# hkchengrex/Cutie

Hardware: AMD Instinct MI355X
Metric: frames/sec (480p, 3 objects) (higher is better)
Workload: dtype bf16

## Files before the change

### cutie_amd/csrc/conv_pc.hip

```cpp
#include "conv_common.h"

typedef __amdgpu_buffer_rsrc_t rsrc_t;
#define PC_WORD3 0x00020000
#define PC_RECORDS 0x7fffffff
#define PC_OOB 0x80000000u
#define LDS_PTR(p) ((__attribute__((address_space(3))) void*)(p))
#define PC_WAIT_VM(N) __builtin_amdgcn_s_waitcnt(((N) & 15) | (((N) >> 4) << 14) | (7 << 4) | (15 << 8))
#define PC_WAIT_LGKM0() __builtin_amdgcn_s_waitcnt(15 | (3 << 14) | (7 << 4) | (0 << 8))
#define PC_BARRIER() { asm volatile("" ::: "memory"); __builtin_amdgcn_s_barrier(); asm volatile("" ::: "memory"); }
#ifdef PC_ABL_NO_LOOPBAR
#define PC_LOOP_BARRIER() { asm volatile("" ::: "memory"); }
#else
#define PC_LOOP_BARRIER() PC_BARRIER()
#endif
#ifdef PC_ABL_NO_WAIT
#define PC_LOOP_WAIT_VM(N) ((void)0)
#else
#define PC_LOOP_WAIT_VM(N) PC_WAIT_VM(N)
#endif
#ifdef PC_ABL_SAME_TILE
#define PC_SAME_TILE_GUARD(...)
#else
#define PC_SAME_TILE_GUARD(...) __VA_ARGS__
#endif
#ifdef PC_ABL_NO_DMA
#define PC_DMA(...) ((void)0)
#else
#define PC_DMA(...) __builtin_amdgcn_raw_ptr_buffer_load_lds(__VA_ARGS__)
#endif

__device__ __forceinline__ rsrc_t pc_rsrc(const void* base) {
    return __builtin_amdgcn_make_buffer_rsrc(const_cast<void*>(base), 0, PC_RECORDS, PC_WORD3);
}

typedef short pc_s16x2 __attribute__((ext_vector_type(2)));
__device__ __forceinline__ unsigned pc_relu2(unsigned w) {
    return __builtin_bit_cast(unsigned, __builtin_elementwise_max(__builtin_bit_cast(pc_s16x2, w), (pc_s16x2){0, 0}));
}

__device__ __forceinline__ int pc_wrow(int R, bool pair) {
    if (!pair) return R;
    const int ii = R & 15, alo = (R >> 4) & 1;
    return (R & ~31) | ((ii >> 2) << 3) | (alo << 2) | (ii & 3);
}

#define PC_HT(TH, TW) ((TH) * 256 + (TW))
template <int BM, int BN, int NS, int HT>
constexpr int pc_lds_bytes(int NPW) {
    if (HT == 0) return NS * (BM + BN) * 128;
    const int TH = HT >> 8, TW = HT & 255, npiece = ((TH + 2) * (TW + 2) + 7) / 8, nxp = (npiece + NPW - 1) / NPW;
    return 2 * nxp * NPW * 1024 + NS * BN * 128;
}

template <int NCH>
__device__ __forceinline__ void pc_finish(const ConvParams& p, float (&v)[NCH], int m, int ch0, bool vec_ok, bool have_res,
                                          const unsigned (&rpre)[NCH / 2], float (&stored)[NCH]) {
#ifdef PC_ABL_FIXED_EPI
    {
#pragma unroll
        for (int r = 0; r < NCH; ++r) v[r] = fmaxf(v[r], 0.f);
        bf16_t* yp = reinterpret_cast<bf16_t*>(p.y) + (long)m * p.ldy + ch0;
        unsigned o[NCH / 2];
#pragma unroll
        for (int r = 0; r < NCH / 2; ++r) o[r] = pack_bf2(v[2 * r], v[2 * r + 1]);
        if constexpr (NCH == 8) *reinterpret_cast<uint4*>(yp) = make_uint4(o[0], o[1], o[NCH / 2 - 2], o[NCH / 2 - 1]);
        else *reinterpret_cast<uint2*>(yp) = make_uint2(o[0], o[1]);
        return;
    }
#endif
    const int act = (p.flags >> CUTIE_ACT_SHIFT) & 7;
    const bool out_f32 = p.flags & CUTIE_F_OUT_F32;
    const bool full = ch0 + NCH <= p.Cout;
    if (p.res) {
        if (have_res) {
#pragma unroll
            for (int r = 0; r < NCH / 2; ++r) { v[2 * r] += __uint_as_float(rpre[r] << 16); v[2 * r + 1] += __uint_as_float(rpre[r] & 0xffff0000u); }
        } else {
            const int mres = conv_res_row(p, m);
            const bf16_t* rp = p.res + (long)mres * p.ldr + ch0;
            if (full && vec_ok) {
                unsigned rr[NCH / 2];
                if constexpr (NCH == 8) { const uint4 t = *reinterpret_cast<const uint4*>(rp); rr[0] = t.x; rr[1] = t.y; rr[NCH / 2 - 2] = t.z; rr[NCH / 2 - 1] = t.w; }
                else { const uint2 t = *reinterpret_cast<const uint2*>(rp); rr[0] = t.x; rr[1] = t.y; }
#pragma unroll
// ... 148 lines not shown
                    }
                }
            }
        }
        if (GAPJ) {
            int c; bool writer;
            const long long tot = pc_colsum16<NCH>(gs, l15, c, writer);
            if (writer) pc_gap_add(p, gap_obj, chbase + a * (PAIR ? 32 : 16) + c, tot);
        }
    }
}

template <int BM, int BN, int WM, int WN, int NPW, int NS, int HT, bool TAPS, bool RELU, bool TWO, int KP = 1>
__global__ __launch_bounds__((WM * WN + NPW) * 64) void conv_pc_kernel(ConvParams p) {
#if __HIP_DEVICE_COMPILE__
    if (p.flags & CUTIE_F_PRIO) __builtin_amdgcn_s_setprio(1);
    constexpr bool HALO = HT > 0;
    constexpr int TH = HALO ? (HT >> 8) : 1, TW = HALO ? (HT & 255) : 1;
    constexpr int NC = WM * WN, NTC = NC * 64;
    constexpr int TM = BM / WM / 16, TN = BN / WN / 16;
    constexpr bool PAIR = (TN % 2) == 0;
    constexpr int NCH = PAIR ? 8 : 4, TNP = PAIR ? TN / 2 : TN;
    constexpr int NXI = HALO ? 1 : BM / 8 / NPW;
    constexpr int NWI = BN / 8 / NPW;
    constexpr int LPT = HALO ? NWI : NXI + NWI;
    constexpr int PH = TH + 2, PW = TW + 2;
    constexpr int NPIECE = (PH * PW + 7) / 8, NXP = (NPIECE + NPW - 1) / NPW, XBUF = NXP * NPW * 1024;
    constexpr int WSTAGE = BN * 128, STAGE = HALO ? WSTAGE : (BM + BN) * 128;
    constexpr int WBASE = HALO ? 2 * XBUF : 0;
    constexpr bool PRE_RES = TM * TNP <= 4;
    static_assert(TM >= 1 && TN >= 1 && BM % (WM * 16) == 0 && BN % (WN * 16) == 0 && NWI >= 1 && NWI * 8 * NPW == BN && NS >= 2 && NS <= 8, "bad tile");
    static_assert(HALO || (NXI >= 1 && NXI * 8 * NPW == BM), "bad stream tile");
    static_assert(!HALO || (TH * TW <= BM && TH * TW > BM - 16 * WM && (NS == 3 || NS == 4) && NXP <= 11 - NS && NXP <= 8), "bad halo tile");
    static_assert(KP == 1 || (KP == 2 && (NS == 4 || NS == 6)), "pair steps: a ring of 2 or 3 pairs");
    constexpr int NP = NS / 2;
    extern __shared__ __attribute__((aligned(16))) u32x4 pc_smem[];
    char* const lds = reinterpret_cast<char*>(pc_smem);
    const int tid = threadIdx.x, lane = tid & 63, l15 = lane & 15, l4 = lane >> 4;
    const int wave = __builtin_amdgcn_readfirstlane(tid >> 6);
    TL_DECL(lds + pc_lds_bytes<BM, BN, NS, HT>(NPW))
    TL(0)
    conv_preload_args(p);
    TL(10)
    const int nb = gridDim.x * gridDim.y;
    int logical;
    {
        const int id = blockIdx.y * gridDim.x + blockIdx.x;
        const int xcd = id & 7, kq = id >> 3, q = nb >> 3, r = nb & 7;
        logical = (xcd < r ? xcd * (q + 1) : r * (q + 1) + (xcd - r) * q) + kq;
    }
    const int mt = logical / (int)gridDim.y;
    const int n0 = (logical - mt * (int)gridDim.y) * BN;
    int m0 = 0, bimg = 0, ty0 = 0, tx0 = 0;
    if (HALO) {
        const int tiles_x = (p.W + TW - 1) / TW, tiles_y = (p.H + TH - 1) / TH, per = tiles_x * tiles_y;
        bimg = mt / per;
        const int r = mt - bimg * per, ty = r / tiles_x;
        ty0 = ty * TH;
        tx0 = (r - ty * tiles_x) * TW;
    } else {
        m0 = mt * BM;
    }
    if (p.zero) {
        const int nthr = (NC + NPW) * 64;
        for (int z = (blockIdx.y * gridDim.x + blockIdx.x) * nthr + tid; z < p.nzero; z += gridDim.x * gridDim.y * nthr) p.zero[z] = 0ull;
    }
    const int nslice = p.Cin / 64;
#ifdef PC_ABL_NO_LOOP
    const int nk = 0;
#else
    const int nk = HALO ? nslice * 9 : p.KH * p.KW * nslice;
#endif

// ... 140 lines not shown
#undef PCS_WPIECE
#undef PCS_XPIECE
        } else {
            unsigned xo1[NXP], xo2[NXP];
#pragma unroll
            for (int i = 0; i < NXP; ++i) {
                const int pp = (pw + NPW * i) * 8 + lr;
                const int py = pp / PW, px = pp - py * PW;
                const int gy = ty0 - 1 + py, gx = tx0 - 1 + px;
                const bool ok = pp < PH * PW && (unsigned)gy < (unsigned)p.H && (unsigned)gx < (unsigned)p.W;
                const unsigned pix = (unsigned)((bimg * p.H + gy) * p.W + gx);
                const unsigned kc = (unsigned)(((lane & 7) ^ (pp & 7)) * 16);
                xo1[i] = ok ? pix * (unsigned)(p.ldx1 * 2) + kc : PC_OOB;
                xo2[i] = TWO ? (ok ? pix * (unsigned)(p.ldx2 * 2) + kc : PC_OOB) : 0u;
            }
            const rsrc_t rx1 = pc_rsrc(p.x1), rx2 = TWO ? pc_rsrc(p.x2) : rx1;
            const int cin2 = p.Cin * 2;
#define PCH_XPIECE(I, SL)                                                                                      \
    {                                                                                                          \
        const bool f_ = !TWO || (SL) * 64 < p.C1;                                                              \
        const int so_ = (f_ ? (SL) * 64 : (SL) * 64 - p.C1) * 2;                                               \
        PC_DMA(f_ ? rx1 : rx2, LDS_PTR(lds + ((SL) & 1) * XBUF + (pw + NPW * (I)) * 1024), 16, f_ ? xo1[I] : xo2[I], so_, 0, 0); \
    }
            int wsl = 0, wtap = 0, wld = 0;
            unsigned wso = 0;
#define PCH_WTILE()                                                                                            \
    {                                                                                                          \
        _Pragma("unroll") for (int i = 0; i < NWI; ++i) PC_DMA(rw, LDS_PTR(lds + wld + wdst + i * 1024), 16, woff[i], wso, 0, 0); \
        wld = wld == (NS - 1) * WSTAGE ? 0 : wld + WSTAGE;                                                     \
        ++wtap; PC_SAME_TILE_GUARD(wso += (unsigned)cin2;)                                                     \
        if (wtap == 9) { wtap = 0; ++wsl; PC_SAME_TILE_GUARD(wso = (unsigned)(wsl * 128);) }                                       \
    }
            TL(1)
#pragma unroll
            for (int s = 0; s < NS - 1; ++s)
                if (s < nk) PCH_WTILE()
#pragma unroll
            for (int i = 0; i < NXP; ++i) PCH_XPIECE(i, 0)
            PC_WAIT_VM(0);
            TL(2)
            PC_BARRIER()
            if constexpr (KP == 1) {
            int sl = 0, tap = 0;
            int xprev = 0;
            int kt = 0;
            for (; kt < nk - (NS - 1); ++kt) {
                TL(3)
                const int xp = (sl + 1 < nslice && tap < NXP) ? 1 : 0;
                if (xp) {
                    switch (tap) {
                        case 0: if constexpr (NXP > 0) PCH_XPIECE(0, sl + 1) break;
                        case 1: if constexpr (NXP > 1) PCH_XPIECE(NXP > 1 ? 1 : 0, sl + 1) break;
                        case 2: if constexpr (NXP > 2) PCH_XPIECE(NXP > 2 ? 2 : 0, sl + 1) break;
                        case 3: if constexpr (NXP > 3) PCH_XPIECE(NXP > 3 ? 3 : 0, sl + 1) break;
                        case 4: if constexpr (NXP > 4) PCH_XPIECE(NXP > 4 ? 4 : 0, sl + 1) break;
                        case 5: if constexpr (NXP > 5) PCH_XPIECE(NXP > 5 ? 5 : 0, sl + 1) break;
                        case 6: if constexpr (NXP > 6) PCH_XPIECE(NXP > 6 ? 6 : 0, sl + 1) break;
                        default: if constexpr (NXP > 7) PCH_XPIECE(NXP > 7 ? 7 : 0, sl + 1) break;
                    }
                }
                PCH_WTILE()
                TL(4)
                const int xin = NS == 3 ? xp : xp + xprev;
                if (xin == 0) { PC_LOOP_WAIT_VM((NS - 2) * NWI); } else if (xin == 1) { PC_LOOP_WAIT_VM((NS - 2) * NWI + 1); } else { PC_LOOP_WAIT_VM((NS - 2) * NWI + 2); }
                TL(5)
                PC_LOOP_BARRIER()
                xprev = xp;
                ++tap;
                if (tap == 9) { tap = 0; ++sl; }
            }
            for (; kt < nk; ++kt) {
                PC_WAIT_VM(0);
                PC_LOOP_BARRIER()
            }
            } else {
// ... 96 lines not shown
            for (int a = 0; a < TNP; ++a) {
                const int ch0 = n0 + cn0 + a * (PAIR ? 32 : 16) + l4 * NCH;
#pragma unroll
                for (int r = 0; r < NCH / 2; ++r) rpre[b][a][r] = 0u;
                if (have_res && mval[b] && ch0 + NCH <= p.Cout) {
                    const int mres = pc_res_row(p, mrow[b]);
                    const bf16_t* rp = p.res + (long)mres * p.ldr + ch0;
                    if constexpr (NCH == 8) { const uint4 t = *reinterpret_cast<const uint4*>(rp); rpre[b][a][0] = t.x; rpre[b][a][1] = t.y; rpre[b][a][NCH / 2 - 2] = t.z; rpre[b][a][NCH / 2 - 1] = t.w; }
                    else { const uint2 t = *reinterpret_cast<const uint2*>(rp); rpre[b][a][0] = t.x; rpre[b][a][1] = t.y; }
                }
            }
    }
    TL(12)
    const int c0 = l4 << 4, c1 = (4 + l4) << 4;
    const int swl = (l15 & 7) << 4;
    int rdw0, rdx0 = 0;
    rdw0 = (HALO ? 0 : BM * 128) + (cn0 + l15) * 128;
    if (!HALO) rdx0 = (pm0 + l15) * 128;
    f32x4 acc[TN][TM];
#pragma unroll
    for (int a = 0; a < TN; ++a)
#pragma unroll
        for (int b = 0; b < TM; ++b) acc[a][b] = (f32x4){0.f, 0.f, 0.f, 0.f};

#ifdef PC_ABL_NO_MFMA
#define PC_MFMA(AF, BF, ACC) ACC[0] += __uint_as_float(__builtin_bit_cast(u32x4, AF).x ^ __builtin_bit_cast(u32x4, BF).y)
#else
#define PC_MFMA(AF, BF, ACC) ACC = __builtin_amdgcn_mfma_f32_16x16x32_bf16(AF, BF, ACC, 0, 0, 0)
#endif
#define PC_RELU4(V) { V.x = pc_relu2(V.x); V.y = pc_relu2(V.y); V.z = pc_relu2(V.z); V.w = pc_relu2(V.w); }
    int rd = 0;
    int sl = 0, tap = 0, toff = 0;
    TL(1)
    PC_BARRIER()
    TL(2)
    for (int kt = 0; kt < nk; ++kt) {
        TL(3)
        u32x4 x0[TM], x1[TM];
        bf16x8 w0[TN], w1[TN];
#ifdef PC_ABL_NO_READ
#pragma unroll
        for (int a = 0; a < TN; ++a) { u32x4 v = {(unsigned)rd + a, (unsigned)lane, 5u, 1u}; w0[a] = __builtin_bit_cast(bf16x8, v); v.w = 2u; w1[a] = __builtin_bit_cast(bf16x8, v); }
#pragma unroll
        for (int b = 0; b < TM; ++b) { x0[b] = (u32x4){(unsigned)rd + b, (unsigned)lane, 3u, 1u}; x1[b] = (u32x4){(unsigned)rd + b, (unsigned)lane, 3u, 2u}; }
#else
        const char* const wst = lds + WBASE + rd + rdw0;
#pragma unroll
        for (int a = 0; a < TN; ++a) {
            w0[a] = __builtin_bit_cast(bf16x8, *reinterpret_cast<const u32x4*>(wst + a * 2048 + (c0 ^ swl)));
            w1[a] = __builtin_bit_cast(bf16x8, *reinterpret_cast<const u32x4*>(wst + a * 2048 + (c1 ^ swl)));
        }
        if (HALO) {
            const char* const xs = lds + (sl & 1) * XBUF;
#pragma unroll
            for (int b = 0; b < TM; ++b) {
                const int pp = xbase[b] + toff;
                const int sw = (pp & 7) << 4;
                x0[b] = *reinterpret_cast<const u32x4*>(xs + pp * 128 + (c0 ^ sw));
                x1[b] = *reinterpret_cast<const u32x4*>(xs + pp * 128 + (c1 ^ sw));
            }
        } else {
            const char* const xs = lds + rd + rdx0;
#pragma unroll
            for (int b = 0; b < TM; ++b) {
                x0[b] = *reinterpret_cast<const u32x4*>(xs + b * 2048 + (c0 ^ swl));
                x1[b] = *reinterpret_cast<const u32x4*>(xs + b * 2048 + (c1 ^ swl));
            }
        }
#endif
        if (RELU) {
#pragma unroll
            for (int b = 0; b < TM; ++b) { PC_RELU4(x0[b]) PC_RELU4(x1[b]) }
        }
#pragma unroll
        for (int a = 0; a < TN; ++a)
#pragma unroll
            for (int b = 0; b < TM; ++b) PC_MFMA(w0[a], __builtin_bit_cast(bf16x8, x0[b]), acc[a][b]);
#pragma unroll
        for (int a = 0; a < TN; ++a)
#pragma unroll
            for (int b = 0; b < TM; ++b) PC_MFMA(w1[a], __builtin_bit_cast(bf16x8, x1[b]), acc[a][b]);
        TL(4)
        if (KP == 1 || (kt & 1) || kt == nk - 1) {
            PC_WAIT_LGKM0();
            PC_LOOP_BARRIER()
        }
        rd = rd == (NS - 1) * STAGE ? 0 : rd + STAGE;
        if (HALO) {
            ++tap;
            toff += (tap == 3 || tap == 6) ? PW - 2 : 1;
            if (tap == 9) { tap = 0; toff = 0; ++sl; }
        }
    }
    TLE(5)
#ifdef PC_ABL_NO_EPILOGUE
    if (acc[0][0][0] != 12345.678f) { TL_DUMP(logical, nb, NC + NPW) return; }
#endif
    int gap_obj = bimg;
    bool gap_one = true;
    if (p.gap && !HALO) {
        const int mf = m0 + pm0, ml = min(mf + BM / WM - 1, p.M - 1);
        const float rd = __builtin_amdgcn_rcpf((float)p.OHW);
        gap_obj = pc_div(min(mf, p.M - 1), p.OHW, rd);
        gap_one = pc_div(ml, p.OHW, rd) == gap_obj;
    }
#ifndef PC_ABL_GENERIC_EPI
    {
        const int act_ = (p.flags >> CUTIE_ACT_SHIFT) & 7;
        const bool gapfast = p.gap && gap_one && !act_ && !p.res && !out_f32;
        if (vec_ok && n0 + BN <= p.Cout && (!p.gap || gapfast) && act_ <= CUTIE_ACT_RELU && !(out_f32 && (act_ || p.res))) {
            const int chbase = n0 + cn0 + l4 * NCH;
#define PC_FAST(RL, F, RS) pc_epilogue_fast<NCH, TM, TNP, PAIR, RL, F, RS, PRE_RES>(p, acc, bias, mrow, mval, chbase, rpre)
            if (gapfast) pc_epilogue_fast<NCH, TM, TNP, PAIR, false, false, false, PRE_RES, true>(p, acc, bias, mrow, mval, chbase, rpre, gap_obj, l15);
            else if (out_f32) PC_FAST(false, true, false);
            else if (p.res) { if (act_) PC_FAST(true, false, true); else PC_FAST(false, false, true); }
            else { if (act_) PC_FAST(true, false, false); else PC_FAST(false, false, false); }
#undef PC_FAST
            TLE(6)
            TL_DUMP(logical, nb, NC + NPW)
            return;
        }
    }
#endif
#pragma unroll
    for (int a = 0; a < TNP; ++a) {
// ... 36 lines not shown
                            for (int pass = 0; pass < 2; ++pass) {
                                const int oo = pass ? o2 : o1;
                                if (pass && !rest) break;
                                long long part[NCH];
#pragma unroll
                                for (int r = 0; r < NCH; ++r) part[r] = (live && ob == oo) ? pc_gapfx(st[r]) : 0;
                                int c; bool writer;
                                const long long tot = pc_colsum16<NCH>(part, l15, c, writer);
                                if (writer) pc_gap_add(p, oo, ch0 + c, tot);
                            }
                        }
                    }
                }
            }
#endif
        }
#ifndef PC_ABL_FIXED_EPI
        if (p.gap && gap_one) {
            int c; bool writer;
            const long long tot = pc_colsum16<NCH>(gsum, l15, c, writer);
            if (writer) pc_gap_add(p, gap_obj, n0 + cn0 + a * (PAIR ? 32 : 16) + l4 * NCH + c, tot);
        }
#endif
    }
    TLE(6)
    TL_DUMP(logical, nb, NC + NPW)
#undef PC_RELU4
#undef PC_MFMA
#endif
}

template <int BM, int BN, int WM, int WN, int NPW, int NS, int HT, bool TAPS, bool RELU, bool TWO, int KP>
static int launch_pc3(const ConvParams& p, hipStream_t s) {
    constexpr int lds = pc_lds_bytes<BM, BN, NS, HT>(NPW) + TL_BYTES;
    static_assert(lds <= 160 * 1024, "LDS");
    static bool attr_set = false;
    if (!attr_set) {
        if (lds > 65536 && hipFuncSetAttribute(reinterpret_cast<const void*>(conv_pc_kernel<BM, BN, WM, WN, NPW, NS, HT, TAPS, RELU, TWO, KP>),
                                               hipFuncAttributeMaxDynamicSharedMemorySize, lds) != hipSuccess) {
            cutie_set_error("conv pc tile: cannot raise the dynamic LDS limit to %d bytes", lds);
            return -2;
        }
        attr_set = true;
    }
    unsigned gx;
    if (HT > 0) {
        constexpr int TH = HT > 0 ? (HT >> 8) : 1, TW = HT > 0 ? (HT & 255) : 1;
        gx = (unsigned)(p.B * ((p.H + TH - 1) / TH) * ((p.W + TW - 1) / TW));
    } else {
        gx = (unsigned)((p.M + BM - 1) / BM);
    }
    hipLaunchKernelGGL((conv_pc_kernel<BM, BN, WM, WN, NPW, NS, HT, TAPS, RELU, TWO, KP>), dim3(gx, (unsigned)((p.Cout + BN - 1) / BN)),
                       dim3((WM * WN + NPW) * 64), lds, s, p);
    return (int)hipGetLastError();
}

template <int BM, int BN, int WM, int WN, int NPW, int NS, int HT, int KP = 1>
static int launch_pc(ConvParams p, hipStream_t s) {
    const long x1_bytes = (long)p.B * p.H * p.W * p.ldx1 * 2, x2_bytes = p.C2 ? (long)p.B * p.H * p.W * p.ldx2 * 2 : 0;
    const long gy = (p.Cout + BN - 1) / BN, w_bytes = gy * BN * (long)p.Kpad * 2;
    if (p.Cin % 64 || (p.C2 && p.C1 % 64) || p.KH > 5 || p.KW > 5 || p.splitk != 1 || p.Kpad < p.KH * p.KW * p.Cin ||
        x1_bytes >= PC_RECORDS - 8192 || x2_bytes >= PC_RECORDS - 8192 || w_bytes >= PC_RECORDS - 8192) {
        cutie_set_error("conv pc tile: needs Cin %% 64 == 0 (C1 too for two sources), KH, KW <= 5, no split-K, operands < 2 GiB "
                        "(Cin=%d C1=%d Kpad=%d k=%dx%d splitk=%d)", p.Cin, p.C1, p.Kpad, p.KH, p.KW, p.splitk);
        return -2;
    }
    if (HT > 0 && (p.KH != 3 || p.KW != 3 || p.stride != 1 || p.pad != 1 || p.OH != p.H || p.OW != p.W)) {
        cutie_set_error("conv pc halo tile: needs 3x3 / stride 1 / pad 1 (k=%dx%d stride=%d pad=%d)", p.KH, p.KW, p.stride, p.pad);
        return -2;
    }
    p.Kslice = p.KH * p.KW * p.Cin;
    const bool relu = p.flags & CUTIE_F_RELU_IN, two = p.C2 != 0, taps = p.pad > 0 || p.KH * p.KW > 1;
#define PC_GO(T_, R_, W_) return launch_pc3<BM, BN, WM, WN, NPW, NS, HT, T_, R_, W_, KP>(p, s)
    if constexpr (HT > 0) {
        if (relu) { if (two) PC_GO(true, true, true); PC_GO(true, true, false); }
        if (two) PC_GO(true, false, true);
        PC_GO(true, false, false);
    } else {
        if (taps) {
            if (relu) { if (two) PC_GO(true, true, true); PC_GO(true, true, false); }
            if (two) PC_GO(true, false, true);
            PC_GO(true, false, false);
        }
        if (relu) { if (two) PC_GO(false, true, true); PC_GO(false, true, false); }
        if (two) PC_GO(false, false, true);
        PC_GO(false, false, false);
    }
#undef PC_GO
}

int launch_conv_pc(const ConvParams& p, int tile, hipStream_t s) {
    switch (tile) {
        case 100: return launch_pc<64, 64, 2, 2, 4, 3, 0>(p, s);
#ifndef PC_QUICK
        case 101: return launch_pc<64, 64, 2, 2, 4, 4, 0>(p, s);
        case 102: return launch_pc<32, 64, 2, 2, 4, 4, 0>(p, s);
        case 103: return launch_pc<128, 64, 2, 2, 4, 3, 0>(p, s);
        case 104: return launch_pc<64, 128, 2, 2, 4, 3, 0>(p, s);
        case 105: return launch_pc<128, 128, 2, 2, 4, 3, 0>(p, s);
        case 106: return launch_pc<128, 128, 2, 2, 8, 3, 0>(p, s);
        case 107: return launch_pc<64, 64, 2, 2, 8, 3, 0>(p, s);
        case 108: return launch_pc<128, 128, 2, 4, 8, 3, 0>(p, s);
        case 109: return launch_pc<32, 64, 2, 2, 4, 6, 0>(p, s);
        case 110: return launch_pc<96, 64, 2, 2, 4, 3, 0>(p, s);
        case 111: return launch_pc<96, 128, 2, 2, 4, 3, 0>(p, s);
#endif
        case 120: return launch_pc<64, 64, 2, 2, 4, 3, PC_HT(8, 8)>(p, s);
#ifndef PC_QUICK
        case 121: return launch_pc<64, 64, 2, 2, 4, 3, PC_HT(4, 16)>(p, s);
        case 122: return launch_pc<128, 64, 2, 2, 4, 3, PC_HT(8, 16)>(p, s);
        case 123: return launch_pc<128, 128, 2, 2, 4, 3, PC_HT(8, 16)>(p, s);
        case 124: return launch_pc<64, 128, 2, 2, 4, 3, PC_HT(8, 8)>(p, s);
        case 125: return launch_pc<32, 64, 2, 2, 4, 3, PC_HT(4, 8)>(p, s);
        case 126: return launch_pc<128, 128, 2, 4, 8, 3, PC_HT(8, 16)>(p, s);
        case 127: return launch_pc<64, 128, 2, 2, 4, 3, PC_HT(4, 16)>(p, s);
        case 129: return launch_pc<96, 64, 2, 2, 4, 3, PC_HT(10, 9)>(p, s);
        case 130: return launch_pc<32, 64, 2, 2, 4, 3, PC_HT(5, 6)>(p, s);
        case 131: return launch_pc<64, 128, 2, 2, 4, 3, PC_HT(6, 9)>(p, s);
        case 132: return launch_pc<64, 64, 2, 2, 4, 3, PC_HT(6, 9)>(p, s);
        case 133: return launch_pc<96, 128, 2, 2, 4, 3, PC_HT(10, 9)>(p, s);
        case 134: return launch_pc<320, 64, 4, 2, 8, 3, PC_HT(20, 16)>(p, s);
        case 140: return launch_pc<64, 64, 2, 2, 4, 4, 0, 2>(p, s);
        case 141: return launch_pc<96, 64, 2, 2, 4, 4, 0, 2>(p, s);
        case 142: return launch_pc<96, 64, 2, 2, 4, 6, 0, 2>(p, s);
        case 143: return launch_pc<32, 64, 2, 2, 4, 4, 0, 2>(p, s);
        case 144: return launch_pc<128, 64, 2, 2, 4, 4, 0, 2>(p, s);
        case 145: return launch_pc<96, 64, 2, 2, 4, 4, PC_HT(10, 9), 2>(p, s);
        case 146: return launch_pc<128, 64, 2, 2, 4, 4, PC_HT(8, 16), 2>(p, s);
        case 147: return launch_pc<32, 64, 2, 2, 4, 4, PC_HT(5, 6), 2>(p, s);
#endif
        default: cutie_set_error("conv: bad pc tile id %d", tile); return -2;
    }
}
```

### cutie_amd/model/plans.py

```python
import math
import os

import numpy as np
import torch

from .. import _lib
from .. import ops as O
from ..ops import Dyn
from .param_spec import resnet_layers

BF16, F32 = torch.bfloat16, torch.float32


class Act:
    __slots__ = ('t', 'B', 'H', 'W', 'C', 'ld')

    def __init__(self, t, B, H, W, C, ld=None):
        self.t, self.B, self.H, self.W, self.C, self.ld = t, B, H, W, C, (C if ld is None else ld)


def positional_encoding(h, w, dim_total, scale, temperature):
    dim = int(math.ceil(dim_total / 4) * 2)
    inv_freq = 1.0 / (temperature ** (torch.arange(0, dim, 2).float() / dim))
    py = torch.arange(h, dtype=torch.float32)
# ... 281 lines not shown
            fl = int(arr['flags'][n])
            key = O.conv_tile_key(M, cout, cin, int(i[11]), int(i[13]), fl & O.F_RELU_IN, fl & O.F_OUT_F32, int(i[1]), int(i[2]))
            best = cache.get(key)
            twin = self.korder_ref and int(i[0]) % self.korder_ref == 0
            kref = self.kref.get(n)
            twin = twin or kref is not None
            if twin:
                M1 = M // self.korder_ref if kref is None else M * kref // int(i[0])
                key1 = (M1,) + key[1:]
                ref = cache.get(key1) or (O.static_tile(M1, cout, cin, int(i[11]), int(i[4]), cout1=int(i[17]) == O.COUT1_TILE), 1)
                want = O.korder_class(*ref)
                if isinstance(want, str) and cache.get(key + (want,)) is not None:
                    best = cache[key + (want,)]
                if best is None or O.korder_class(*best) != want:
                    best = (int(i[17]), 1) if O.korder_class(int(i[17]), int(i[19])) == want else tuple(ref)
                assert O.korder_class(*best) == want, (key, best, ref)
            if best is None and not getattr(self.eng, 'autotune', AUTOTUNE):
                continue
            if best is None:
                one = arr[n:n + 1].copy()
                best, best_t = (int(i[17]), 1), None
                cands = O.tile_candidates(M, cout, cin, int(i[16]),
                                          geom=dict(kh=int(i[11]), stride=int(i[13]), pad=int(i[14]), W=int(i[2]), c2=int(i[4])))
                if int(i[4]) or arr['p'][n, 4]:
                    cands = [t for t in cands if t != O.COUT1_TILE]
                for t in cands:
                    for sk in O.splitk_candidates(M, cout, int(i[16]), t):
                        one['i'][0, 17], one['i'][0, 19] = t, sk
                        ms = min(ex.time_ops(one, TUNE_ITERS) for _ in range(TUNE_REPS))
                        if best_t is None or ms < best_t:
                            best, best_t = (t, sk), ms
                cache[key] = best
                tuned_any = True
            apply = True
            if (best[0] in O.DMA_TILES or best[0] in O.PC_TILES) and not O.dma_tiles_enabled():
                apply = False
            if (arr['p'][n, 7] or arr['p'][n, 8]) and best[0] not in O.DMA_TILES and best[0] not in O.PC_TILES:
                apply = False
            if apply:
                arr['i'][n, 17], arr['i'][n, 19] = best
            if twin:
                assert O.korder_class(int(arr['i'][n, 17]), int(arr['i'][n, 19])) == want, (key, int(arr['i'][n, 17]), int(arr['i'][n, 19]), want)
        ol.wire_next_weights()
        self.tuned = True
        if tuned_any:
            save_tile_cache(cache)

    def conv(self, wname, x, *, name=None, out=None, stride=1, pad=None, x2=None, res=None, res_bcast=False,
             relu_in=False, act=O.ACT_NONE, out_f32=False, ldy=None, gap_acc=None, zero=None, persistent=False, res_group=None):
        w = self.eng.w[wname]
        if pad is None:
            pad = (w.kh - 1) // 2
        OH = (x.H + 2 * pad - w.kh) // stride + 1
        OW = (x.W + 2 * pad - w.kw) // stride + 1
        if out is None:
            t = self.buf(name or wname, (x.B, OH, OW, w.cout), F32 if out_f32 else BF16, persistent=persistent)
            out = Act(t, x.B, OH, OW, w.cout, w.cout if ldy is None else ldy)
        else:
            assert out.B == x.B and out.H == OH and out.W == OW and out.C == w.cout, (wname, out.B, out.H, out.W, out.C, OH, OW, w.cout)
        if res is not None:
            assert res.C == w.cout and res.H == OH and res.W == OW

        def emit(s0, s1, zero):
            whole = s0 == 0 and s1 == x.B
            cut = (lambda a, elem: a.t) if whole else (lambda a, elem: _objects_from(a, s0, elem))
            return self.ol.conv(cut(x, 2), w, cut(out, 4 if out_f32 else 2), B=s1 - s0, H=x.H, W=x.W, C1=x.C, ldx1=x.ld, OH=OH, OW=OW, ldy=out.ld, stride=stride,
# ... 456 lines not shown
```

### cutie_amd/model/weights.py

```python
import torch

BN_EPS = 1e-5


class PackedConv:
    __slots__ = ('weight', 'bias', 'cout', 'cin_padded', 'kh', 'kw', 'kpad', 'cin_real')

    def __init__(self, weight, bias, cout, cin_padded, kh, kw, kpad, cin_real=None):
        self.weight, self.bias, self.cout, self.cin_padded = weight, bias, cout, cin_padded
        self.kh, self.kw, self.kpad = kh, kw, kpad
        self.cin_real = cin_padded if cin_real is None else cin_real


class PackedLinear:
    __slots__ = ('weight', 'bias', 'n', 'kd')

    def __init__(self, weight, bias, n, kd):
        self.weight, self.bias, self.n, self.kd = weight, bias, n, kd


def fold_bn(w, sd, bn):
    g, b = sd[bn + '.weight'].float(), sd[bn + '.bias'].float()
    m, v = sd[bn + '.running_mean'].float(), sd[bn + '.running_var'].float()
    s = g / torch.sqrt(v + BN_EPS)
    return w * s.view(-1, 1, 1, 1), b - m * s


def pack_conv(w, bias, device, segs=None):
    w = w.float()
    cout, cin, kh, kw = w.shape
    if segs is None:
        segs = [(cin, -(-cin // 8) * 8)]
    assert sum(r for r, _ in segs) == cin
    parts, c0 = [], 0
    for real, padded in segs:
        assert padded % 8 == 0 and padded >= real
        part = w[:, c0:c0 + real]
        if padded > real:
            part = torch.cat([part, torch.zeros(cout, padded - real, kh, kw)], 1)
        parts.append(part)
        c0 += real
    w = torch.cat(parts, 1)
    cin_p = w.shape[1]
    k = kh * kw * cin_p
    kpad = -(-k // 128) * 128
    coutpad = -(-cout // 128) * 128
    flat = w.permute(0, 2, 3, 1).reshape(cout, k)
    packed = torch.zeros(coutpad, kpad)
    packed[:cout, :k] = flat
    return PackedConv(packed.to(torch.bfloat16).to(device).contiguous(),
                      None if bias is None else bias.float().to(device).contiguous(), cout, cin_p, kh, kw, kpad, cin_real=cin)


def pack_linear(w, bias, device):
    w = w.float()
    n, kd = w.shape
    assert kd % 8 == 0
    return PackedLinear(w.to(torch.bfloat16).to(device).contiguous(),
                        None if bias is None else bias.float().to(device).contiguous(), n, kd)


def linear_as_conv(w, bias, device):
    return pack_conv(w.float().view(w.shape[0], w.shape[1], 1, 1), bias, device)


def out_proj_blob(w):
    assert w.cout == 256 and w.kh == 1 and w.kw == 1 and w.cin_padded == 256 and w.bias is not None
    return torch.cat([w.weight[:256, :256].contiguous().view(torch.uint8).reshape(-1), w.bias.contiguous().view(torch.uint8).reshape(-1)]).contiguous()
```

### cutie_amd/ops.py

```python
import os

import numpy as np
import torch

from . import _lib

NI, NF, NP = 24, 6, 16
OP_DTYPE = np.dtype([('kind', '<i4'), ('flags', '<i4'), ('i', '<i4', (NI,)), ('f', '<f4', (NF,)), ('p', '<u8', (NP,))])
assert OP_DTYPE.itemsize == _lib.OP_STRUCT_SIZE

(CONV, MAXPOOL, IMG_PREP, UPSAMPLE2X_ADD, AREA_DOWN, MASK_DOWN, GAP, ECA_APPLY, GRU, SEG_AGG, UP4_SOFTMAX,
 MASK_MERGE, AGG_SOFTMAX, LINEAR, LAYERNORM, QUERY_INIT, AUX_MASK, ATTN_Q2P, ATTN_SELF, ATTN_P2Q, SUMMARIZE,
 ADD_PE, KEY_PREP, AFF_SCORE, AFF_SELECT, AFF_READOUT, MEMSET32, COPY2D, AXPY, USAGE_TICK, RANK_SELECT,
 GATHER_ROWS, CONSOL_AFF, CONSOL_READ, CAST, PROB_TO_ID, RESIZE, FLIP_W, AREA_DOWN3, QFFN, STEM, BANK_WRITE) = range(1, 43)

KIND_NAMES = {}
for _n in ('CONV MAXPOOL IMG_PREP UPSAMPLE2X_ADD AREA_DOWN MASK_DOWN GAP ECA_APPLY GRU SEG_AGG UP4_SOFTMAX MASK_MERGE '
           'AGG_SOFTMAX LINEAR LAYERNORM QUERY_INIT AUX_MASK ATTN_Q2P ATTN_SELF ATTN_P2Q SUMMARIZE ADD_PE KEY_PREP '
           'AFF_SCORE AFF_SELECT AFF_READOUT MEMSET32 COPY2D AXPY USAGE_TICK RANK_SELECT GATHER_ROWS CONSOL_AFF '
           'CONSOL_READ CAST PROB_TO_ID RESIZE FLIP_W AREA_DOWN3 QFFN STEM').split():
    KIND_NAMES[globals()[_n]] = _n

F_RELU_IN, F_OUT_F32, F_RES_BCAST = 1, 2, 4
F_PRIO, F_AFF_PRIO = 256, 64
F_TILE_OFF = 128 if os.environ.get('CUTIE_AMD_COUT1_TILE', '1') in ('', '0') else 0
ACT_NONE, ACT_RELU, ACT_SIGMOID, ACT_SQ1 = 0, 1, 2, 3
ACT_SHIFT = 4
AREA_RT = 8 if os.environ.get('CUTIE_AMD_AREA_R', '1') in ('', '0') else 0
GRU_SCALAR = 1 if os.environ.get('CUTIE_AMD_GRU4', '1') in ('', '0') else 0
KEYPREP_LOOP = 2 if os.environ.get('CUTIE_AMD_KEYPREP_LOOP', '0') not in ('', '0') else 0
UP4_LANES = 16 if os.environ.get('CUTIE_AMD_UP4_SHARED', '1') in ('', '0') else 0
SELECT_COARSE = 2 if os.environ.get('CUTIE_AMD_SELECT_FINE', '1') in ('', '0') else 0
UP4_RTK = 8 if os.environ.get('CUTIE_AMD_UP4_KC', '1') in ('', '0') else 0

TILES = {0: (128, 128, 32), 1: (128, 64, 32), 2: (64, 64, 32), 3: (256, 16, 32), 4: (64, 128, 32),
         5: (64, 64, 64), 6: (64, 128, 64), 7: (128, 128, 64), 8: (64, 64, 128), 9: (32, 64, 64),
         10: (128, 64, 64), 11: (32, 64, 128), 12: (32, 128, 64),
         13: (64, 64, 64), 14: (128, 64, 64), 15: (64, 128, 64), 16: (128, 128, 64), 17: (64, 64, 128), 18: (128, 128, 32),
         20: (64, 64, 64), 21: (64, 64, 128), 22: (32, 64, 128), 23: (128, 64, 64), 24: (64, 128, 64), 25: (128, 128, 64),
         26: (32, 64, 64), 27: (64, 64, 64), 28: (32, 64, 64), 29: (64, 128, 32), 30: (64, 64, 32)}
TILE_WK = {20: 2, 21: 2, 22: 2, 23: 2, 24: 2, 25: 2, 26: 2, 27: 4, 28: 4, 29: 2, 30: 2}

DMA_TILES = {60: (128, 128, 64), 61: (128, 128, 64), 62: (128, 128, 64), 63: (128, 64, 64), 64: (64, 128, 64), 65: (64, 64, 64),
             66: (64, 64, 64), 67: (32, 64, 64), 68: (256, 128, 64), 69: (32, 128, 64), 70: (128, 128, 64), 71: (128, 64, 64),
             72: (64, 64, 64), 73: (64, 64, 64), 74: (64, 64, 64), 75: (32, 64, 64), 76: (128, 64, 64), 77: (64, 128, 64), 78: (32, 128, 64),
             80: (64, 64, 128), 81: (64, 64, 128), 82: (32, 64, 128), 83: (32, 64, 128), 84: (64, 128, 128), 85: (128, 64, 128),
             86: (96, 64, 64), 87: (96, 64, 64), 88: (64, 64, 64), 89: (64, 64, 64)}


PC_TILES = {100: (64, 64, 64), 101: (64, 64, 64), 102: (32, 64, 64), 103: (128, 64, 64), 104: (64, 128, 64), 105: (128, 128, 64),
            106: (128, 128, 64), 107: (64, 64, 64), 108: (128, 128, 64), 109: (32, 64, 64), 110: (96, 64, 64), 111: (96, 128, 64),
            120: (64, 64, 64), 121: (64, 64, 64), 122: (128, 64, 64), 123: (128, 128, 64), 124: (64, 128, 64), 125: (32, 64, 64),
            126: (128, 128, 64), 127: (64, 128, 64), 129: (96, 64, 64), 130: (32, 64, 64), 131: (64, 128, 64),
            132: (64, 64, 64), 133: (96, 128, 64), 134: (320, 64, 64),
            140: (64, 64, 64), 141: (96, 64, 64), 142: (96, 64, 64), 143: (32, 64, 64), 144: (128, 64, 64),
            145: (96, 64, 64), 146: (128, 64, 64), 147: (32, 64, 64)}
PC_HALO = {120: (8, 8), 121: (4, 16), 122: (8, 16), 123: (8, 16), 124: (8, 8), 125: (4, 8), 126: (8, 16), 127: (4, 16),
           129: (10, 9), 130: (5, 6), 131: (6, 9), 132: (6, 9), 133: (10, 9), 134: (20, 16),
           145: (10, 9), 146: (8, 16), 147: (5, 6)}

ALL_TILES = {**TILES, **DMA_TILES, **PC_TILES}


def korder_class(tile, splitk=1):
    if tile in PC_HALO:
        return 'halo'
    if tile in TILE_WK or splitk != 1:
        return ('split', tile, splitk)
    if tile in (3, COUT1_TILE):
        return ('small', tile)
    return 'stream' if (tile in DMA_TILES or tile in PC_TILES) else 'igemm'


def pc_tile_ok(tile, *, cin, kh, stride=1, pad=None, c2=0):
    if cin % 64 or (c2 and (c2 % 64 or (cin - c2) % 64)) or kh > 5:
        return False
    if tile in PC_HALO:
        return kh == 3 and stride == 1 and (pad is None or pad == 1)
    return True


def pc_blocks(tile, B, OH, OW, cout):
    bm, bn, _ = PC_TILES[tile]
    if tile in PC_HALO:
        th, tw = PC_HALO[tile]
        return B * -(-OH // th) * -(-OW // tw) * -(-cout // bn)
    return -(-(B * OH * OW) // bm) * -(-cout // bn)


def dma_tiles_enabled():
    return os.environ.get('CUTIE_AMD_DMA_TILES', '1') not in ('', '0')

# ... 13 lines not shown


COUT1_TILE = 19


def cout1_ok(cout, cin, c2=0, res=False):
    lp = cin // 8
    return cout == 1 and c2 == 0 and not res and cin % 8 == 0 and 1 <= lp <= 64 and (lp & (lp - 1)) == 0


def tile_candidates(M, cout, cin, kpad=None, geom=None):
    if cout <= 16:
        return [3] + ([COUT1_TILE] if cout1_ok(cout, cin) else [])
    out = []
    for t, (bm, bn, bk) in TILES.items():
        if t == 3 or (bk > 32 and cin < 32):
            continue
        wk = TILE_WK.get(t, 1)
        if wk > 1 and (kpad is None or (kpad // bk) % wk or kpad // bk < 2 * wk):
            continue
        if bn == 128 and cout <= 64:
            continue
        if bm * 2 > max(M, 64) * 2 and bm > 64:
            continue
        out.append(t)
    if dma_tiles_enabled() and geom is not None and dma_tile_ok(60, cin=cin, kh=geom['kh'], c2=geom.get('c2', 0)):
        for t, (bm, bn, bk) in DMA_TILES.items():
            if not (bn == 128 and cout <= 64) and not (bm > 64 and bm > max(M, 64)) and not (bm == 256 and M < 16384) \
                    and dma_tile_ok(t, cin=cin, kh=geom['kh'], c2=geom.get('c2', 0)):
                out.append(t)
    if dma_tiles_enabled() and geom is not None:
        for t, (bm, bn, bk) in PC_TILES.items():
            if pc_tile_ok(t, cin=cin, kh=geom['kh'], stride=geom.get('stride', 1), pad=geom.get('pad'), c2=geom.get('c2', 0)) \
                    and not (bn == 128 and cout <= 64) and not (bm > 64 and bm > max(M, 64)) and not (bm == 256 and M < 16384):
                out.append(t)
    return out


SPLITK_PART_FLOATS = 16 << 20
_splitk_scratch = {}


def splitk_scratch(device, owner=None):
    dev = torch.device(device)
    store = _splitk_scratch if owner is None else owner.__dict__.setdefault('_splitk_part', {})
    key = str(dev)
    if key not in store:
        n = SPLITK_PART_FLOATS if dev.type == 'cuda' else 1024
        store[key] = torch.zeros(n, dtype=torch.float32, device=device)
    return store[key]


def splitk_candidates(M, cout, kpad, tile):
    if tile == COUT1_TILE or tile == 3 or tile in DMA_TILES or tile in PC_TILES:
        return [1]
    bm, bn, bk = TILES[tile]
    blocks = -(-M // bm) * -(-cout // bn)
    nk = kpad // bk // TILE_WK.get(tile, 1)
    ldp = (cout + 7) & ~7
    out = [1]
    for sk in (2, 3, 4, 6, 8, 9, 12, 16, 18):
        if blocks >= NUM_CU or blocks * sk > 6 * NUM_CU or nk // sk < 2:
            break
        if sk * M * ldp > SPLITK_PART_FLOATS:
            break
        if nk % sk == 0:
            out.append(sk)
# ... 134 lines not shown

    def finalize(self):
        arr = np.zeros(len(self.recs), dtype=OP_DTYPE)
        for n, (kind, flags, ints, floats, ptrs) in enumerate(self.recs):
            arr['kind'][n] = kind
            arr['flags'][n] = flags
            arr['i'][n, :len(ints)] = ints
            arr['f'][n, :len(floats)] = floats
            arr['p'][n, :len(ptrs)] = ptrs
        self.arr = arr
        self._words = None
        self.wire_next_weights()
        return arr

    def wire_next_weights(self):
        arr = self.arr
        convs = [n for n in range(len(arr)) if arr['kind'][n] == CONV]
        for n in convs:
            arr['p'][n, 9:11] = 0
            arr['i'][n, 22:24] = 0
        if not (WEIGHT_PREFETCH and self.touch_next_weights):
            return
        nxt, nxt2 = None, None
        for n in reversed(convs):
            i = arr['i'][n]
            pc = int(i[17]) in PC_TILES
            if nxt is not None and pc:
                budget = WEIGHT_PREFETCH_BLOCK * -(-pc_blocks(int(i[17]), int(i[0]), int(i[7]), int(i[8]), int(i[9])) // 8)
                n1 = min(nxt[1], WEIGHT_PREFETCH, budget)
                arr['p'][n, 9], arr['i'][n, 22] = nxt[0], n1
                n2 = min(nxt2[1], WEIGHT_PREFETCH, budget - n1) if (nxt2 is not None and not nxt[2]) else 0
                if n2 > 0:
                    arr['p'][n, 10], arr['i'][n, 23] = nxt2[0], n2
            nxt, nxt2 = (int(arr['p'][n, 2]), self.wbytes[n], pc), nxt

    def patch_ints(self, op, start, values):
        values = [int(v) for v in values]
        ints = self.recs[op][2]
        end = start + len(values)
        if len(ints) < end:
            ints.extend([0] * (end - len(ints)))
        ints[start:end] = values
        if self.arr is not None:
            self.arr['i'][op, start:end] = values

    def bind(self, **tensors):
        if self.arr is None:
            self.finalize()
        words = self._words
        if words is None:
            assert OP_DTYPE.itemsize == 256 and OP_DTYPE.fields['p'][1] == 128
            words = self._words = ({name: tuple((idx * 32 + 16 + slot, off) for (idx, slot, off) in sl) for name, sl in self.dyn.items()},
                                   memoryview(self.arr).cast('B').cast('Q'))
        table, mv = words
        for name, t in tensors.items():
            sl = table.get(name)
            if sl is None:
                continue
            base = 0 if t is None else (t if type(t) is int else t.data_ptr())
            if base:
                for w, off in sl:
                    mv[w] = base + off
            else:
                for w, off in sl:
                    mv[w] = 0

    def run(self, _stream=None, **tensors):
        if self.arr is None:
            self.finalize()
        if tensors:
            self.bind(**tensors)
        ex = _lib.get_executor()
        if _stream is None:
            ex.run(self.arr)
        elif hasattr(ex, 'run_on'):
            ex.run_on(self.arr, _stream)
        else:
            with torch.cuda.stream(_stream):
                ex.run(self.arr)

    def __len__(self):
        return len(self.recs)

    def conv(self, x1, w, y, *, B, H, W, C1, ldx1, OH, OW, ldy, stride=1, pad=0, x2=None, C2=0, ldx2=0,
             res=None, ldr=0, res_bcast=False, relu_in=False, act=ACT_NONE, out_f32=False, tile=None, splitk=1,
             gap_acc=None, zero=None, prio=False, res_group=None):
        flags = (F_RELU_IN if relu_in else 0) | (F_OUT_F32 if out_f32 else 0) | (F_RES_BCAST if res_bcast else 0) | (act << ACT_SHIFT) | F_TILE_OFF | \
            (F_PRIO if prio else 0)
        assert C1 + C2 == w.cin_padded, (C1, C2, w.cin_padded)
        M = B * OH * OW
        side = gap_acc is not None or zero is not None
        if tile is None:
            tile = static_tile(M, w.cout, C1 + C2, w.kh, C2, res is not None, side)
        if side:
            assert (tile in DMA_TILES or tile in PC_TILES) and not out_f32 and w.cout % 8 == 0 and ldy % 8 == 0, 'GAP accumulation needs an LDS-DMA conv (see conv_side_jobs_ok)'
        part = splitk_scratch(w.weight.device, self.scratch_owner)
        self.wbytes[len(self.recs)] = w.weight.numel() * w.weight.element_size()
        return self.add(CONV, flags,
                        [B, H, W, C1, C2, ldx1, ldx2, OH, OW, w.cout, ldy, w.kh, w.kw, stride, pad, ldr, w.kpad, tile, w.cin_real,
                         splitk, part.numel() // 1024, 0 if zero is None else zero.numel()],
                        self._res_group(res_group, res_bcast, B, OH * OW), [x1, x2, w.weight, w.bias, res, y, part, gap_acc, zero])

    @staticmethod
    def _res_group(res_group, res_bcast, B, OHW):
        if res_group is None:
            return []
        kg, stride = int(res_group[0]), int(res_group[1])
        assert res_bcast and kg > 0 and B % kg == 0 and stride >= OHW and stride < (1 << 24), (res_group, B, OHW)
        return [float(kg), float(stride)]

    def maxpool(self, x, y, *, B, H, W, C, relu=False):
        OH, OW = (H + 2 - 3) // 2 + 1, (W + 2 - 3) // 2 + 1
        return self.add(MAXPOOL, 1 if relu else 0, [B, H, W, C, OH, OW], [], [x, y])

    STEM_MAX_IMAGES = 12

    def stem(self, image, masks, w, y, *, h0, w0, H, W, pad_left, pad_top, K, mean, std, relu=True, more_images=(), mask_stride=0, counts=None):
        assert w.cout == 64 and w.kh == 7 and w.cin_padded == 8 and H % 16 == 0 and W % 16 == 0
        more = list(more_images)
        assert len(more) < self.STEM_MAX_IMAGES
        if counts is not None:
            assert len(counts) == 1 + len(more) and len(counts) > 1
            ints = [h0, w0, H, W, pad_left, pad_top, max(counts), w.kpad, len(counts), 0, pack_counts(counts)]
            return self.add(STEM, 1 if relu else 0, ints, list(mean) + list(std), [image, masks, w.weight, w.bias, y] + more)
        ints = [h0, w0, H, W, pad_left, pad_top, K, w.kpad] + ([1 + len(more), int(mask_stride)] if more else [])
        return self.add(STEM, 1 if relu else 0, ints, list(mean) + list(std), [image, masks, w.weight, w.bias, y] + more)
# ... 648 lines not shown
```

Baseline: 1172.

## Add halo conv tiles that stream weights into registers from a fragment-ordered copy

Adds halo-tile variants (150-152) of the pipelined 3x3 conv in which each wave loads its weight fragments straight from global memory into registers, using a second fragment-ordered copy stored after the packed weights. LDS then holds only the double-buffered input halo, which drops the weight staging ring and its per-tap barriers in favour of one barrier per input-channel slice. The costs are more register pressure, doubled weight memory for 3x3 convs, and global-load latency that now has to be hidden by the NS-deep register ring. The new tiles become autotune candidates by default, and the weight-prefetch hints are updated to point at the fragment copy.

```diff
diff --git a/cutie_amd/csrc/conv_pc.hip b/cutie_amd/csrc/conv_pc.hip
--- a/cutie_amd/csrc/conv_pc.hip
+++ b/cutie_amd/csrc/conv_pc.hip
@@ -45,11 +45,11 @@
 }
 
 #define PC_HT(TH, TW) ((TH) * 256 + (TW))
-template <int BM, int BN, int NS, int HT>
+template <int BM, int BN, int NS, int HT, int KP = 1>
 constexpr int pc_lds_bytes(int NPW) {
     if (HT == 0) return NS * (BM + BN) * 128;
     const int TH = HT >> 8, TW = HT & 255, npiece = ((TH + 2) * (TW + 2) + 7) / 8, nxp = (npiece + NPW - 1) / NPW;
-    return 2 * nxp * NPW * 1024 + NS * BN * 128;
+    return 2 * nxp * NPW * 1024 + (KP == 9 ? 0 : NS * BN * 128);
 }
 
 template <int NCH>
@@ -264,13 +264,14 @@
     static_assert(TM >= 1 && TN >= 1 && BM % (WM * 16) == 0 && BN % (WN * 16) == 0 && NWI >= 1 && NWI * 8 * NPW == BN && NS >= 2 && NS <= 8, "bad tile");
     static_assert(HALO || (NXI >= 1 && NXI * 8 * NPW == BM), "bad stream tile");
     static_assert(!HALO || (TH * TW <= BM && TH * TW > BM - 16 * WM && (NS == 3 || NS == 4) && NXP <= 11 - NS && NXP <= 8), "bad halo tile");
-    static_assert(KP == 1 || (KP == 2 && (NS == 4 || NS == 6)), "pair steps: a ring of 2 or 3 pairs");
+    static_assert(KP == 1 || (KP == 2 && (NS == 4 || NS == 6)) || (KP == 9 && HALO && NS == 3 && PAIR), "pair steps: a ring of 2 or 3 pairs; slice steps: halo tiles");
+    constexpr bool WREG = KP == 9;
     constexpr int NP = NS / 2;
     extern __shared__ __attribute__((aligned(16))) u32x4 pc_smem[];
     char* const lds = reinterpret_cast<char*>(pc_smem);
     const int tid = threadIdx.x, lane = tid & 63, l15 = lane & 15, l4 = lane >> 4;
     const int wave = __builtin_amdgcn_readfirstlane(tid >> 6);
-    TL_DECL(lds + pc_lds_bytes<BM, BN, NS, HT>(NPW))
+    TL_DECL(lds + pc_lds_bytes<BM, BN, NS, HT, KP>(NPW))
     TL(0)
     conv_preload_args(p);
     TL(10)
@@ -477,15 +478,27 @@
         if (wtap == 9) { wtap = 0; ++wsl; PC_SAME_TILE_GUARD(wso = (unsigned)(wsl * 128);) }                                       \
     }
             TL(1)
+            if constexpr (!WREG) {
 #pragma unroll
             for (int s = 0; s < NS - 1; ++s)
                 if (s < nk) PCH_WTILE()
+            }
 #pragma unroll
             for (int i = 0; i < NXP; ++i) PCH_XPIECE(i, 0)
             PC_WAIT_VM(0);
             TL(2)
             PC_BARRIER()
-            if constexpr (KP == 1) {
+            if constexpr (WREG) {
+            for (int sl = 1; sl < nslice; ++sl) {
+                TL(3)
+#pragma unroll
+                for (int i = 0; i < NXP; ++i) PCH_XPIECE(i, sl)
+                TL(4)
+                PC_WAIT_VM(0);
+                TL(5)
+                PC_LOOP_BARRIER()
+            }
+            } else if constexpr (KP == 1) {
             int sl = 0, tap = 0;
             int xprev = 0;
             int kt = 0;
@@ -648,6 +661,72 @@
     int rd = 0;
     int sl = 0, tap = 0, toff = 0;
     TL(1)
+    if constexpr (WREG) {
+        typedef const __attribute__((address_space(1))) u32x4* pc_gv4;
+        typedef const __attribute__((address_space(1))) char* pc_gch;
+        const int nstep = nslice * 9;
+        const long wmat = (long)((p.Cout + 127) & ~127) * p.Kpad * 2;
+        const pc_gch wf0 = (pc_gch)reinterpret_cast<const char*>(p.w) + wmat;
+        unsigned wlane[TN];
+#pragma unroll
+        for (int a = 0; a < TN; ++a) wlane[a] = (unsigned)(((n0 + cn0) / 16 + a) * nstep) * 2048u + (unsigned)lane * 16u;
+        u32x4 wr[NS][TN][2];
+        int wnext = 0;
+        const int wlast = (nstep - 1) * 2048;
+#define PCW_LOAD(SLOT)                                                                                         \
+    {                                                                                                          \
+        _Pragma("unroll") for (int a = 0; a < TN; ++a) {                                                       \
+            wr[SLOT][a][0] = *(pc_gv4)(wf0 + wnext + wlane[a]);                                                \
+            wr[SLOT][a][1] = *(pc_gv4)(wf0 + wnext + wlane[a] + 1024);                                         \
+        }                                                                                                      \
+        wnext = min(wnext + 2048, wlast);                                                                      \
+    }
+#pragma unroll
+        for (int s = 0; s < NS; ++s) PCW_LOAD(s)
+        PC_BARRIER()
+        TL(2)
+        for (int s = 0; s < nslice; ++s) {
+            const char* const xs = lds + (s & 1) * XBUF;
+            u32x4 xc[2][TM], xn[2][TM];
+#define PCW_XREAD(DST, TOFF)                                                                                   \
+    _Pragma("unroll") for (int b = 0; b < TM; ++b) {                                                           \
+        const int pp = xbase[b] + (TOFF);                                                                      \
+        const int o0 = pp * 128 + (c0 ^ ((pp & 7) << 4));                                                      \
+        DST[0][b] = *reinterpret_cast<const u32x4*>(xs + o0);                                                  \
+        DST[1][b] = *reinterpret_cast<const u32x4*>(xs + (o0 ^ 64));                         \
+    }
+            PCW_XREAD(xc, 0)
+#pragma unroll
+            for (int t = 0; t < 9; ++t) {
+                TL(3)
+                if (t < 8) { PCW_XREAD(xn, ((t + 1) / 3) * PW + (t + 1) % 3) }
+                if (RELU) {
+#pragma unroll
+                    for (int b = 0; b < TM; ++b) { PC_RELU4(xc[0][b]) PC_RELU4(xc[1][b]) }
+                }
+#pragma unroll
+                for (int h = 0; h < 2; ++h)
+#pragma unroll
+                    for (int a = 0; a < TN; ++a)
+#pragma unroll
+                        for (int b = 0; b < TM; ++b)
+                            PC_MFMA(__builtin_bit_cast(bf16x8, wr[t % NS][a][h]), __builtin_bit_cast(bf16x8, xc[h][b]), acc[a][b]);
+                PCW_LOAD(t % NS)
+                __builtin_amdgcn_sched_barrier(0);
+                if (t < 8) {
+#pragma unroll
+                    for (int b = 0; b < TM; ++b) { xc[0][b] = xn[0][b]; xc[1][b] = xn[1][b]; }
+                }
+                TL(4)
+            }
+            if (s + 1 < nslice) {
+                PC_WAIT_LGKM0();
+                PC_LOOP_BARRIER()
+            }
+        }
+#undef PCW_XREAD
+#undef PCW_LOAD
+    } else {
     PC_BARRIER()
     TL(2)
     for (int kt = 0; kt < nk; ++kt) {
@@ -707,6 +786,7 @@
             toff += (tap == 3 || tap == 6) ? PW - 2 : 1;
             if (tap == 9) { tap = 0; toff = 0; ++sl; }
         }
+    }
     }
     TLE(5)
 #ifdef PC_ABL_NO_EPILOGUE
@@ -809,7 +889,7 @@
 
 template <int BM, int BN, int WM, int WN, int NPW, int NS, int HT, bool TAPS, bool RELU, bool TWO, int KP>
 static int launch_pc3(const ConvParams& p, hipStream_t s) {
-    constexpr int lds = pc_lds_bytes<BM, BN, NS, HT>(NPW) + TL_BYTES;
+    constexpr int lds = pc_lds_bytes<BM, BN, NS, HT, KP>(NPW) + TL_BYTES;
     static_assert(lds <= 160 * 1024, "LDS");
     static bool attr_set = false;
     if (!attr_set) {
@@ -866,6 +946,17 @@
 #undef PC_GO
 }
 
+#ifdef PC_WREG_UNIT
+int launch_conv_pc_wreg(const ConvParams& p, int tile, hipStream_t s) {
+    switch (tile) {
+        case 150: return launch_pc<96, 64, 2, 2, 4, 3, PC_HT(10, 9), 9>(p, s);
+        case 151: return launch_pc<32, 64, 2, 2, 4, 3, PC_HT(5, 6), 9>(p, s);
+        case 152: return launch_pc<128, 64, 2, 2, 4, 3, PC_HT(8, 16), 9>(p, s);
+        default: cutie_set_error("conv: bad pc tile id %d", tile); return -2;
+    }
+}
+#else
+int launch_conv_pc_wreg(const ConvParams& p, int tile, hipStream_t s);
 int launch_conv_pc(const ConvParams& p, int tile, hipStream_t s) {
     switch (tile) {
         case 100: return launch_pc<64, 64, 2, 2, 4, 3, 0>(p, s);
@@ -883,6 +974,7 @@
         case 111: return launch_pc<96, 128, 2, 2, 4, 3, 0>(p, s);
 #endif
         case 120: return launch_pc<64, 64, 2, 2, 4, 3, PC_HT(8, 8)>(p, s);
+        case 150: case 151: case 152: return launch_conv_pc_wreg(p, tile, s);
 #ifndef PC_QUICK
         case 121: return launch_pc<64, 64, 2, 2, 4, 3, PC_HT(4, 16)>(p, s);
         case 122: return launch_pc<128, 64, 2, 2, 4, 3, PC_HT(8, 16)>(p, s);
@@ -909,3 +1001,4 @@
         default: cutie_set_error("conv: bad pc tile id %d", tile); return -2;
     }
 }
+#endif
diff --git a/cutie_amd/csrc/conv_pc_wreg.hip b/cutie_amd/csrc/conv_pc_wreg.hip
--- /dev/null
+++ b/cutie_amd/csrc/conv_pc_wreg.hip
@@ -0,0 +1,2 @@
+#define PC_WREG_UNIT
+#include "conv_pc.hip"
diff --git a/cutie_amd/model/plans.py b/cutie_amd/model/plans.py
--- a/cutie_amd/model/plans.py
+++ b/cutie_amd/model/plans.py
@@ -337,6 +337,7 @@
                             best, best_t = (t, sk), ms
                 cache[key] = best
                 tuned_any = True
+            best = (O.wreg_resolve(best[0]), best[1])
             apply = True
             if (best[0] in O.DMA_TILES or best[0] in O.PC_TILES) and not O.dma_tiles_enabled():
                 apply = False
diff --git a/cutie_amd/model/weights.py b/cutie_amd/model/weights.py
--- a/cutie_amd/model/weights.py
+++ b/cutie_amd/model/weights.py
@@ -48,8 +48,36 @@
     flat = w.permute(0, 2, 3, 1).reshape(cout, k)
     packed = torch.zeros(coutpad, kpad)
     packed[:cout, :k] = flat
-    return PackedConv(packed.to(torch.bfloat16).to(device).contiguous(),
-                      None if bias is None else bias.float().to(device).contiguous(), cout, cin_p, kh, kw, kpad, cin_real=cin)
+    packed = packed.to(torch.bfloat16)
+    if has_frag_copy(kh, kw, cin_p):
+        both = torch.zeros(2 * coutpad * kpad, dtype=torch.bfloat16)
+        both[:coutpad * kpad] = packed.reshape(-1)
+        frag = packed.reshape(-1)[frag_order_index(coutpad, kpad, cin_p)]
+        both[coutpad * kpad:coutpad * kpad + frag.numel()] = frag
+        packed = both.to(device)[:coutpad * kpad].view(coutpad, kpad)
+    else:
+        packed = packed.to(device).contiguous()
+    return PackedConv(packed, None if bias is None else bias.float().to(device).contiguous(), cout, cin_p, kh, kw, kpad, cin_real=cin)
+
+
+def has_frag_copy(kh, kw, cin_padded):
+    return kh == 3 and kw == 3 and cin_padded % 64 == 0
+
+
+def frag_order_index(coutpad, kpad, cin_padded):
+    assert coutpad % 32 == 0 and cin_padded % 64 == 0 and 9 * cin_padded <= kpad
+    nslice = cin_padded // 64
+    R = torch.arange(coutpad).view(-1, 1, 1, 1, 1, 1)
+    ii, alo = R & 15, (R >> 4) & 1
+    row = (R & ~31) | ((ii >> 2) << 3) | (alo << 2) | (ii & 3)
+    sl = torch.arange(nslice).view(1, -1, 1, 1, 1, 1)
+    tap = torch.arange(9).view(1, 1, -1, 1, 1, 1)
+    half = torch.arange(2).view(1, 1, 1, -1, 1, 1)
+    chunk = torch.arange(4).view(1, 1, 1, 1, -1, 1)
+    e = torch.arange(8).view(1, 1, 1, 1, 1, -1)
+    src = row * kpad + tap * cin_padded + sl * 64 + half * 32 + chunk * 8 + e
+    src = src.view(coutpad // 16, 16, nslice, 9, 2, 4, 8).permute(0, 2, 3, 4, 5, 1, 6)
+    return src.reshape(-1)
 
 
 def pack_linear(w, bias, device):
diff --git a/cutie_amd/ops.py b/cutie_amd/ops.py
--- a/cutie_amd/ops.py
+++ b/cutie_amd/ops.py
@@ -54,10 +54,18 @@
             126: (128, 128, 64), 127: (64, 128, 64), 129: (96, 64, 64), 130: (32, 64, 64), 131: (64, 128, 64),
             132: (64, 64, 64), 133: (96, 128, 64), 134: (320, 64, 64),
             140: (64, 64, 64), 141: (96, 64, 64), 142: (96, 64, 64), 143: (32, 64, 64), 144: (128, 64, 64),
-            145: (96, 64, 64), 146: (128, 64, 64), 147: (32, 64, 64)}
+            145: (96, 64, 64), 146: (128, 64, 64), 147: (32, 64, 64),
+            150: (96, 64, 64), 151: (32, 64, 64), 152: (128, 64, 64)}
 PC_HALO = {120: (8, 8), 121: (4, 16), 122: (8, 16), 123: (8, 16), 124: (8, 8), 125: (4, 8), 126: (8, 16), 127: (4, 16),
            129: (10, 9), 130: (5, 6), 131: (6, 9), 132: (6, 9), 133: (10, 9), 134: (20, 16),
-           145: (10, 9), 146: (8, 16), 147: (5, 6)}
+           145: (10, 9), 146: (8, 16), 147: (5, 6),
+           150: (10, 9), 151: (5, 6), 152: (8, 16)}
+PC_WREG = {150: 129, 151: 130, 152: 122}
+WREG_TILES = os.environ.get('CUTIE_AMD_WREG_TILES', '1') not in ('', '0')
+
+
+def wreg_resolve(tile):
+    return tile if WREG_TILES else PC_WREG.get(tile, tile)
 
 ALL_TILES = {**TILES, **DMA_TILES, **PC_TILES}
 
@@ -137,7 +145,7 @@
     if dma_tiles_enabled() and geom is not None:
         for t, (bm, bn, bk) in PC_TILES.items():
             if pc_tile_ok(t, cin=cin, kh=geom['kh'], stride=geom.get('stride', 1), pad=geom.get('pad'), c2=geom.get('c2', 0)) \
-                    and not (bn == 128 and cout <= 64) and not (bm > 64 and bm > max(M, 64)) and not (bm == 256 and M < 16384):
+                    and (WREG_TILES or t not in PC_WREG) and not (bn == 128 and cout <= 64) and not (bm > 64 and bm > max(M, 64)) and not (bm == 256 and M < 16384):
                 out.append(t)
     return out
 
@@ -338,7 +346,11 @@
                 n2 = min(nxt2[1], WEIGHT_PREFETCH, budget - n1) if (nxt2 is not None and not nxt[2]) else 0
                 if n2 > 0:
                     arr['p'][n, 10], arr['i'][n, 23] = nxt2[0], n2
-            nxt, nxt2 = (int(arr['p'][n, 2]), self.wbytes[n], pc), nxt
+            if int(i[17]) in PC_WREG:
+                frag_bytes = -(-int(i[9]) // 128) * 128 * 9 * (int(i[3]) + int(i[4])) * 2
+                nxt, nxt2 = (int(arr['p'][n, 2]) + self.wbytes[n], frag_bytes, pc), nxt
+            else:
+                nxt, nxt2 = (int(arr['p'][n, 2]), self.wbytes[n], pc), nxt
 
     def patch_ints(self, op, start, values):
         values = [int(v) for v in values]
@@ -398,6 +410,8 @@
         side = gap_acc is not None or zero is not None
         if tile is None:
             tile = static_tile(M, w.cout, C1 + C2, w.kh, C2, res is not None, side)
+        if tile in PC_WREG:
+            assert w.kh == 3 and w.kw == 3 and w.cin_padded % 64 == 0 and stride == 1 and pad == 1, 'weights-in-registers tiles need the fragment-ordered weight copy'
         if side:
             assert (tile in DMA_TILES or tile in PC_TILES) and not out_f32 and w.cout % 8 == 0 and ldy % 8 == 0, 'GAP accumulation needs an LDS-DMA conv (see conv_side_jobs_ok)'
         part = splitk_scratch(w.weight.device, self.scratch_owner)
```

New measurement: 1177 (median of 3 runs). Within noise of the previous version (+0.4%).
